# srogatch/ProbQA

Hardware: AMD Instinct MI355X
Metric: next_question_selections_per_sec (higher is better)
Workload: dtype f64; 1 GPU; 1000Qx5Ax1000T fp64 cube resident in HBM, single in-flight quiz; step = priority sweep + argmax + question id on host, synchronous call through the C ABI; questions_per_gpu=1000, parallelism=single GPU, eval_kernel=wg256_np2, selected_question=500

## Files before the change

probqa_amd/csrc/engine_options.h:

```cpp
#pragma once

#include <cstdint>
#include <cstdio>
#include <cstdlib>
#include <cstring>

#include "pqa_kernels.h"

namespace pqa {

struct EngineOptions {
  int64_t server = 0;
  int64_t serverIdleUs = 500;
  int64_t serverVramMailbox = 1;
  int64_t bugCompat = 1;
  int64_t speculate = 1;
  int64_t fuseUpdate = 1;
  int64_t combine = 1;
  int64_t combineSpin = 1;
  int64_t lingerUs = 20;
  int64_t postAlways = 0;
  int64_t poleFix = 1;
  int64_t poleGate = 1;
  int64_t poleLazy = 1;
  int64_t poleFollow = 1;
  int64_t lateEager = 3;
  int64_t select = 0;
  int64_t workers = 16;
  int64_t evalSubtasks = 0;
  int64_t evalVariant = 0;
  int64_t evalMaxGrid = 0;
  int64_t useGraph = 0;
  int64_t timeSweeps = 0;
  int64_t hostSampled = 1;
  int64_t fusedSampled = 0;
  int64_t sampledBatchHost = 0;
  int64_t batchMin = 0;
  int64_t batchForm = 0;
  int64_t batchQb = 0;
  int64_t batchTile = 0;
  int64_t batchGroups = 0;
  int64_t batchTail = 1;
  int64_t rerank = 1;
  int64_t clusterFrom = 10240;
  int64_t clusterForm = 0;
  int64_t clusterShape = 0;
  int64_t longRowForm = 1;
  int64_t topExact = 1;
  int64_t topCache = 10;
  int64_t rowsStage = 1;
  int64_t trainChunkSteps = int64_t(1) << 22;
};

enum : uint8_t {
// ... 106 lines not shown
```

probqa_amd/csrc/eval_kernels.hip:

```cpp
#include "pqa_device.h"
#include "eval_device.h"
#include "pqa_kernels.h"
#include "prior_device.h"
#include "pole_device.h"

namespace pqa {

static __device__ double gLog2Table[kLog2TableDoubles];
hipError_t UploadLog2Table(const double *hostTable) {
  return hipMemcpyToSymbol(HIP_SYMBOL(gLog2Table), hostTable, kLog2TableDoubles * sizeof(double));
}

struct EvalArgs {
  const double *cube;
  const double *prior;
  const uint32_t *tgap;
  const uint32_t *qgap;
  const uint32_t *asked;
  double *priority;
  double *poleScratch;
  PoleHeader *poleList;
  bool serverWatch;
  bool serverNoWatch;
  int64_t K, T, ldT, qFirst, qLimit;
  double vCompTail;
  FusedSelect fs;
  const QuizSlot *slots;
  int maxGrid;
  int poleNoFollow;
  int poleGate;
  const double *updRowA, *updRowD;
  int64_t updQuestion;
  int64_t updVects, updWorkers;
  int64_t updT;
  TopRequest updTop;
};

__device__ __forceinline__ void select_quiz(EvalArgs &a) {
  if (a.slots == nullptr) return;
  const QuizSlot s = a.slots[blockIdx.y];
  a.prior = s.prior;
  a.asked = s.asked;
  a.priority = s.priority;
  a.fs.out = s.out;
  a.fs.seq = s.seq;
  a.fs.hostPriority = s.hostPriority;
  a.fs.scratch += (size_t)blockIdx.y * (size_t)a.fs.scratchStride;
}

__device__ __forceinline__ void store_priority(double *p, double v) {
  __hip_atomic_store(p, v, __ATOMIC_RELAXED, __HIP_MEMORY_SCOPE_AGENT);
}

// ... 10 lines not shown
}
template <int CTRL>
__device__ __forceinline__ void best_step(Best &b) {
  const double op = mov_dpp<CTRL>(b.p);
  const int64_t oi = mov_dpp_i64<CTRL>(b.i);
  best_merge(b, op, oi);
}
__device__ __forceinline__ Best wave_best(Best b) {
  best_step<kDppXor1>(b);
  best_step<kDppXor2>(b);
  best_step<kDppHalfMirror>(b);
  best_step<kDppMirror>(b);
  Pair p = swap16(b.p);
  PairI64 i = swap16_i64(b.i);
  b = Best{p.a, i.a};
  best_merge(b, p.b, i.b);
  p = swap32(b.p);
  i = swap32_i64(b.i);
  b = Best{p.a, i.a};
  best_merge(b, p.b, i.b);
  return b;
}

template <bool UNI = false>
__device__ __forceinline__ void fused_select(const EvalArgs &a, Best mine, int lane, bool *allReported = nullptr, bool wgSuspect = false) {
  if (a.fs.scratch == nullptr) return;
  const bool sampled = a.fs.sampleSubtasks > 0;
  if (sampled && a.fs.hostPriority == nullptr) asm volatile("s_waitcnt vmcnt(0)" ::: "memory");
  const Best wg = wave_best(mine);
  uint64_t seqValue = a.fs.seqValue, flagValue = a.fs.flagValue;
  if (a.fs.tagCell != nullptr)
    seqValue = flagValue = __hip_atomic_load(a.fs.tagCell, __ATOMIC_RELAXED, __HIP_MEMORY_SCOPE_AGENT);
  const uint64_t tag = (uint64_t)(uint32_t)seqValue << 32;
  SelectResult *rec = a.fs.scratch;
  if (UNI || lane == 0) {
    typedef unsigned int u4 __attribute__((ext_vector_type(4)));
    const uint64_t w0 = d2u(wg.p), w1 = tag | (uint32_t)(wg.i < 0 ? 0x7FFFFFFFu : (uint32_t)wg.i) | (wgSuspect ? 0x80000000u : 0u);
    const u4 v = {(unsigned)w0, (unsigned)(w0 >> 32), (unsigned)w1, (unsigned)(w1 >> 32)};
    asm volatile("global_store_dwordx4 %0, %1, off sc1" ::"v"(rec + blockIdx.x), "v"(v) : "memory");
  }
  if (blockIdx.x != 0) return;
  const unsigned grid = gridDim.x;
  typedef unsigned int u4 __attribute__((ext_vector_type(4)));
  bool complete = true;
  uint32_t anySuspect = 0;
  Best b{0.0, -1};
  for (unsigned chunk = 0; chunk < grid && complete; chunk += 16 * kWave) {
// ... 13 lines not shown
          "s_waitcnt vmcnt(0)"
          : "=&v"(r[0]), "=&v"(r[1]), "=&v"(r[2]), "=&v"(r[3]), "=&v"(r[4]), "=&v"(r[5]), "=&v"(r[6]), "=&v"(r[7]),
            "=&v"(r[8]), "=&v"(r[9]), "=&v"(r[10]), "=&v"(r[11]), "=&v"(r[12]), "=&v"(r[13]), "=&v"(r[14]), "=&v"(r[15])
          : "v"(p0), "v"(p1), "v"(p2), "v"(p3)
          : "memory");
      bool mine = true;
#pragma unroll
      for (int u = 0; u < 16; u++)
        if (chunk + lane + u * kWave < grid) mine = mine && r[u][3] == (unsigned)(tag >> 32);
      all = __all(mine);
      if (!all) __builtin_amdgcn_s_sleep(2);
    }
    complete = all;
#pragma unroll
    for (int u = 0; u < 16; u++)
      if (chunk + lane + u * kWave < grid) {
        const uint64_t pw = (uint64_t)r[u][0] | ((uint64_t)r[u][1] << 32);
        anySuspect |= r[u][2] >> 31;
        best_merge(b, u2d(pw), (r[u][2] & 0x7FFFFFFFu) == 0x7FFFFFFFu ? -1 : (int64_t)(r[u][2] & 0x7FFFFFFFu));
      }
  }
  b = wave_best(b);
  const bool suspects = __any(anySuspect != 0);
  const bool listed = !UNI && suspects && complete && a.poleList != nullptr, lazy = a.fs.lazyFix != 0;
  const bool deferred = listed && !lazy, redo = (UNI && suspects && !a.serverNoWatch) || (listed && lazy);
  if (sampled) {
    if (allReported != nullptr && (UNI || lane == 0)) { allReported[0] = complete; allReported[1] = deferred; allReported[2] = redo; }
    return;
  }
  if (deferred) return;
  if (UNI || lane == 0) {
    if (a.fs.packed) host_publish_packed(a.fs.out, b.i < 0 ? 0.0 : b.p, flagValue, !complete ? -3 : redo ? -4 : b.i < 0 ? -1 : b.i);
    else host_publish(a.fs.out, b.i < 0 ? 0.0 : b.p, !complete ? -3 : redo ? -4 : b.i < 0 ? -1 : b.i + a.fs.outBase, a.fs.seq, flagValue);
    if (a.fs.tagCell != nullptr) {
      uint64_t next = seqValue + 1;
      if ((uint32_t)next == 0) next++;
      __hip_atomic_store(a.fs.tagCell, next, __ATOMIC_RELAXED, __HIP_MEMORY_SCOPE_AGENT);
    }
  }
}


constexpr int kSusDoubles = 4;

constexpr int kPend = 32;

__host__ __device__ constexpr size_t eval_lds_fixed_doubles(int wpq, int64_t K) {
  return kLog2TableDoubles + 2 * (size_t)wpq + 2 * (size_t)(K + 2) * wpq + (size_t)kPend * (2 * (size_t)K + 3) + 2 * kWave + kSusDoubles;
}
static_assert(kSusDoubles % 2 == 0 && kLog2TableDoubles % 2 == 0 && (kPend * 3) % 2 == 0,
              "the LDS priors behind the fixed part are read as 16-byte pairs: an odd count of doubles in front of them halves their rate (10000 x 5 x 10000: 906 -> 1250 us)");
__host__ __device__ constexpr size_t eval_md_row_offset_bytes(int wpq, int64_t K) {
  return (eval_lds_fixed_doubles(wpq, K) * sizeof(double) + 1023) / 1024 * 1024;
}
__host__ __device__ constexpr size_t eval_lds_doubles(int wpq, int64_t K, bool prLds, int64_t ldT) {
  return kLog2TableDoubles + 2 * (size_t)wpq + 2 * (size_t)(K + 2) * wpq + (size_t)kPend * (2 * (size_t)K + 3) + 2 * kWave + kSusDoubles +
         (prLds ? (size_t)ldT + 2 : 0);
}

__host__ __device__ constexpr bool eval_defers_sums(int wpq, int np, bool prLds) { return wpq <= 8 && !(wpq == 2 && np == 4); }
__host__ __device__ constexpr size_t eval_deferred_bytes(int wpq, int np, int64_t K, bool prLds) {
  return eval_defers_sums(wpq, np, prLds) ? (size_t)(K + 2) * wpq * kWave * sizeof(double) : 0;
}

__device__ __forceinline__ void flush_pending(const EvalArgs &a, const double *pend, int nPend, int lane, Best &best) {
  if (lane < nPend) {
    const int64_t K = a.K;
    const double *rec = pend + (size_t)lane * (2 * K + 3);
    const int64_t q = reinterpret_cast<const int64_t *>(rec)[2 * K + 2];
    const double pri = eval_epilogue(rec, -rec[2 * K], rec + K, K, rec[2 * K + 1], a.vCompTail);
    store_priority(a.priority + (q - a.qFirst), pri);
    if (a.fs.hostPriority != nullptr && a.fs.sampleSubtasks > 0) {
      typedef unsigned int u4 __attribute__((ext_vector_type(4)));
      const uint64_t w0 = d2u(pri), w1 = a.fs.seqValue;
      const u4 x = {(unsigned)w0, (unsigned)(w0 >> 32), (unsigned)w1, (unsigned)(w1 >> 32)};
      asm volatile("global_store_dwordx4 %0, %1, off sc0 sc1" ::"v"(a.fs.hostPriority + (q - a.qFirst)), "v"(x) : "memory");
    }
    best_offer(best, pri, q - a.qFirst);
  }
}

__device__ __forceinline__ double uniform_double(double x) {
  const uint64_t u = d2u(x);
  const uint32_t lo = __builtin_amdgcn_readfirstlane((uint32_t)u), hi = __builtin_amdgcn_readfirstlane((uint32_t)(u >> 32));
  return u2d(((uint64_t)hi << 32) | lo);
}
template <bool COH>
__device__ __forceinline__ uint32_t load_word(const uint32_t *p) {
  if constexpr (COH) return __hip_atomic_load(p, __ATOMIC_RELAXED, __HIP_MEMORY_SCOPE_AGENT);
  else return *p;
}
template <bool COH>
__device__ __forceinline__ double2 load_pair(const double2 *p) {
  if constexpr (COH) {
    const double *d = reinterpret_cast<const double *>(p);
    return make_double2(__hip_atomic_load(d, __ATOMIC_RELAXED, __HIP_MEMORY_SCOPE_AGENT),
                        __hip_atomic_load(d + 1, __ATOMIC_RELAXED, __HIP_MEMORY_SCOPE_AGENT));
  } else {
    return *p;
  }
}

template <int WPQ, int NP, bool PRLDS, bool SERVER, bool DEFER, bool FUSE = false, bool POLE = false, int KC = 0>
__device__ __forceinline__ void sweep_body(EvalArgs a, bool copyTable) {
  constexpr int kThreads = WPQ * kWave;
  constexpr int NPR = PRLDS ? 1 : NP;
  constexpr bool kStreamHint = !SERVER && WPQ >= 8;
  extern __shared__ double smem[];
  const int64_t ldT = a.ldT, K = KC > 0 ? KC : a.K;
  double *tbl = smem;
  if (!lds_table_at_zero(tbl)) __builtin_trap();
  double *redW = tbl + kLog2TableDoubles;
  double *partAll = redW + 2 * WPQ;
  double *pend = partAll + 2 * (K + 2) * WPQ;
  Best *bestLds = reinterpret_cast<Best *>(pend + kPend * (2 * K + 3));
  uint32_t *susWords = reinterpret_cast<uint32_t *>(bestLds + kWave);
  double2 *prLds = reinterpret_cast<double2 *>(reinterpret_cast<double *>(bestLds + kWave) + kSusDoubles);
  constexpr bool kMdLds = !PRLDS;
  double2 *mdRow = reinterpret_cast<double2 *>(reinterpret_cast<char *>(smem) + eval_md_row_offset_bytes(WPQ, K));
  const int nPart = (int)(K + 2);
  const int recLen = (int)(2 * K + 3);
  int tidRaw = threadIdx.x;
  if constexpr (SERVER) asm volatile("" : "+v"(tidRaw));
  const int tid = tidRaw, lane = tid % kWave;
  const int wave = SERVER ? (int)__builtin_amdgcn_readfirstlane(tid / kWave) : tid / kWave;
  const unsigned mdRowWaveAddr = (unsigned)(uintptr_t)mdRow + (unsigned)wave * 1024u;
  constexpr bool kDefer = DEFER;
  double *vdump = PRLDS ? reinterpret_cast<double *>(prLds) + ldT + 2
                        : reinterpret_cast<double *>(reinterpret_cast<char *>(mdRow) + (size_t)NP * kThreads * 16);
  const int nPairs = (int)(ldT >> 1);
  const int64_t qStride = (K + 1) * ldT, rowBytes = ldT * 8;
  uint32_t poff[NP];
  uint32_t gapWord[NP];
  double2 pr[NPR], prRaw[NP];
  double2 invD[NP], ring[NP];
  const int64_t q0 = a.qFirst + blockIdx.x;
  const bool haveQ0 = q0 < a.qLimit;
  const int64_t q0c = haveQ0 ? q0 : a.qLimit - 1;
  const uint32_t q0Gap = a.qgap[q0c >> 5], q0Asked = load_word<SERVER>(a.asked + (q0c >> 5));
#pragma unroll
  for (int j = 0; j < NP; j++) {
    const int p = tid + j * kThreads;
    const int pc = p < nPairs ? p : (nPairs - 1);
    poff[j] = (uint32_t)pc * 16u;
    gapWord[j] = a.tgap[pc >> 4];
    prRaw[j] = load_pair<SERVER>(reinterpret_cast<const double2 *>(a.prior) + pc);
  }
  auto head_of_stream = [&](int64_t qq) __attribute__((always_inline)) {
    if constexpr (kMdLds) {
      const RowRsrc rowA = row_rsrc(a.cube + qq * qStride, rowBytes);
      const dma_rsrc_t md = dma_rsrc<true>(a.cube + qq * qStride + K * ldT, rowBytes);
#pragma unroll
      for (int j = 0; j < NP; j++) {
        ring[j] = row_load<kStreamHint>(rowA, poff[j]);
        dma16(md, poff[j], mdRowWaveAddr + (unsigned)j * (kThreads * 16u));
      }
    } else {
      const RowRsrc rowD = row_rsrc(a.cube + qq * qStride + K * ldT, rowBytes);
#pragma unroll
      for (int j = 0; j < NP; j++) ring[j] = row_load<kStreamHint>(rowD, poff[j]);
    }
  };
// ... 36 lines not shown
#pragma unroll
    for (int j = 0; j < NP; j++) {
      const int p = tid + j * kThreads;
      if (p < nPairs) {
        double2 v = make_double2(stage[2 * p], stage[2 * p + 1]);
        if (2 * p < 4 * a.updVects) v.x = v.x / total;
        if (2 * p + 1 < 4 * a.updVects) v.y = v.y / total;
        prRaw[j] = v;
        if (blockIdx.x == gridDim.x - 1) { stage[2 * p] = v.x; stage[2 * p + 1] = v.y; }
      }
    }
    if (blockIdx.x == gridDim.x - 1) {
      if (tid == 0) const_cast<uint32_t *>(a.asked)[a.updQuestion >> 5] |= 1u << (a.updQuestion & 31);
      if (a.updTop.count > 0) {
        __syncthreads();
        top_targets_publish<true>(stage, a.tgap, a.updT, a.updTop.count, a.updTop.out, a.updTop.nOut, a.updTop.flag, a.updTop.flagValue, topScratch);
      }
    }
    __syncthreads();
    double2 *tblDst = reinterpret_cast<double2 *>(tbl);
    tblDst[tid] = tv0; tblDst[tid + kThreads] = tv1; tblDst[tid + 2 * kThreads] = tv2; tblDst[tid + 3 * kThreads] = tv3;
  }
  uint32_t gapBits = 0;
#pragma unroll
  for (int j = 0; j < NP; j++) {
    const int p = tid + j * kThreads;
    const bool inRow = p < nPairs;
    const int sh = (2 * (inRow ? p : nPairs - 1)) & 31;
    const bool g0 = !inRow || ((gapWord[j] >> sh) & 1u), g1 = !inRow || ((gapWord[j] >> (sh + 1)) & 1u);
    gapBits |= (g0 ? 1u : 0u) << (2 * j) | (g1 ? 1u : 0u) << (2 * j + 1);
    double2 pv = prRaw[j];
    pv.x = g0 ? 0.0 : pv.x;
    pv.y = g1 ? 0.0 : pv.y;
    if constexpr (PRLDS) { if (inRow) prLds[p] = pv; } else { pr[j] = pv; }
  }
  if constexpr (PRLDS) { if (tid == 0) prLds[nPairs] = make_double2(0.0, 0.0); }

  auto next_valid = [&](int64_t q) {
    while (q < a.qLimit && (bit_test(a.qgap, q) || ((load_word<SERVER>(a.asked + (q >> 5)) >> (q & 31)) & 1u) || (FUSE && q == a.updQuestion))) {
      if (tid == 0) store_priority(a.priority + (q - a.qFirst), 0.0);
      q += gridDim.x;
    }
    return q;
  };
  if (tid < 4) susWords[tid] = tid < 2 ? 0u : kGapNoneBits;
  int64_t q = q0;
  if (haveQ0 && ((((q0Gap | q0Asked) >> (q0 & 31)) & 1u) || (FUSE && q0 == a.updQuestion))) {
    q = next_valid(q0);
    if (q < a.qLimit) head_of_stream(q);
  }
  __syncthreads();

  int phase = 0, qpar = 0, nPend = 0;
  constexpr bool kWatch = POLE;
  constexpr bool kListWatch = kWatch && !SERVER;
  [[maybe_unused]] int32_t stepNear = INT32_MIN, stepSmall = INT32_MIN;
  const bool watchOn = SERVER ? a.serverWatch : a.poleList != nullptr;
  bool wgSuspect = false;
  if (wave == 0) bestLds[lane] = Best{0.0, -1};
  constexpr bool kHeadInTail = !kMdLds && KC > 0;
  [[maybe_unused]] bool firstOfStream = true;
  auto head_pair = [&](const RowRsrc &rowA, int j) __attribute__((always_inline)) {
    invD[j].x = ((gapBits >> (2 * j)) & 1) ? 0.0 : div_nr(1.0, ring[j].x);
    invD[j].y = ((gapBits >> (2 * j + 1)) & 1) ? 0.0 : div_nr(1.0, ring[j].y);
    ring[j] = row_load<kStreamHint>(rowA, poff[j]);
  };
  auto head_from_ring = [&](const double *qBase) __attribute__((always_inline)) {
    const RowRsrc rowA = row_rsrc(qBase, rowBytes);
#pragma unroll
    for (int j = 0; j < NP; j++) {
      head_pair(rowA, j);
      __builtin_amdgcn_sched_barrier(0);
    }
  };
  while (q < a.qLimit) {
    const int64_t qn = next_valid(q + gridDim.x);
    const double *qBase = a.cube + q * qStride;
    if constexpr (kMdLds) {
      asm volatile("s_waitcnt vmcnt(0)" ::: "memory");
#pragma unroll
      for (int j = 0; j < NP; j++) {
        const double2 dv = mdRow[j * kThreads + tid];
        invD[j].x = ((gapBits >> (2 * j)) & 1) ? 0.0 : div_nr(1.0, dv.x);
        invD[j].y = ((gapBits >> (2 * j + 1)) & 1) ? 0.0 : div_nr(1.0, dv.y);
        __builtin_amdgcn_sched_barrier(0);
      }
    } else if (!kHeadInTail || firstOfStream) {
      head_from_ring(qBase);
      firstOfStream = false;
    }
    double *part = partAll + qpar * (nPart * WPQ);
    double *rec = pend + nPend * recLen;
    double accL = 0, hW = 0;
    [[maybe_unused]] int32_t rowGap = INT32_MIN;
    [[maybe_unused]] uint32_t watchRows = 0;
#pragma unroll KC > 0 ? KC : 1
    for (int64_t k = 0; k < K; k++) {
      double2 lh[NP];
      double s0 = 0, s1 = 0;
      const bool lastRow = k + 1 == K;
      const bool moreQuestions = qn < a.qLimit;
      const double *rowNext = !lastRow ? qBase + (k + 1) * ldT
                              : !moreQuestions ? a.prior
                              : a.cube + qn * qStride + (kMdLds ? 0 : K * ldT);
      const RowRsrc rowN = row_rsrc(rowNext, rowBytes);
#pragma unroll
      for (int j = 0; j < NP; j++) {
// ... 85 lines not shown
        double acc = src[0];
#pragma unroll
        for (int i = 1; i < kGroups; i++) acc += src[32 * i];
        acc += mov_dpp<kDppXor1>(acc);
        acc += mov_dpp<kDppXor2>(acc);
        acc += mov_dpp<kDppHalfMirror>(acc);
        acc += mov_dpp<kDppMirror>(acc);
        const Pair p = swap16(acc);
        acc = p.a + p.b;
        if constexpr (kListWatch) {
          if (l32 == 0 && r < K && acc <= kSmallV && ((wideRows >> (r < 15 ? r : 15)) & 1u)) atomicOr(&susWords[qpar], 1u << (r < 15 ? r : 15));
        }
        if (r < K) acc = rec[r] * sqrt(acc);
        if (l32 == 0) rec[K + r] = acc;
      }
      if constexpr (kListWatch) {
        if (wideRows != 0) { __syncthreads(); suspect = (susWords[qpar] & 0xFFFFu) != 0; }
        if constexpr (!SERVER) { if (a.poleNoFollow) suspect = false; }
      }
      if (tid == 0) {
        reinterpret_cast<int64_t *>(rec)[2 * K + 2] = q;
        if constexpr (kListWatch) { susWords[qpar ^ 1] = 0; susWords[2 + (qpar ^ 1)] = kGapNoneBits; }
        if constexpr (!SERVER) {
          if (suspect) susWords[4] = pole_list_append(a.poleList, (uint32_t)(q - a.qFirst), K <= 15 ? susWords[qpar] & 0xFFFFu : 0u, a.slots != nullptr ? blockIdx.y : 0u,
                                                      a.poleGate ? susWords[2 + qpar] : 0u);
        }
      }
      wgSuspect = wgSuspect || suspect;
      if (!SERVER && suspect) {
        __syncthreads();
        const int64_t at = a.slots != nullptr ? (int64_t)susWords[4] : q - a.qFirst;
        for (int i = tid; i < 2 * (int)K + 2; i += kThreads) a.poleScratch[at * (2 * K + 2) + i] = rec[i];
      }
      if (nPend + 1 == kPend) {
        __syncthreads();
        if (wave == 0) flush_pending(a, pend, kPend, lane, bestLds[lane]);
      }
    } else {
      hW = wave_sum(hW);
      accL = wave_sum(accL);
      if (lane == 0) {
        part[K * WPQ + wave] = hW;
        part[(K + 1) * WPQ + wave] = accL;
      }
      if constexpr (kListWatch) {
        if (watchRows != 0) atomicOr(&susWords[qpar], watchRows);
      }
      if constexpr (WPQ > 1) __syncthreads();
      uint32_t wideRows = 0;
      if constexpr (kListWatch) {
        const uint32_t w = watchOn ? susWords[qpar] : 0u;
        suspect = (w & 0xFFFFu) != 0;
        wideRows = w >> 16;
      }
      if (wave == 0) {
        for (int r = lane; r < nPart; r += kWave) {
          double acc = part[r * WPQ];
          for (int w2 = 1; w2 < WPQ; w2++) acc += part[r * WPQ + w2];
          if constexpr (kListWatch) {
            if (r < K && acc <= kSmallV && ((wideRows >> (r < 15 ? r : 15)) & 1u)) atomicOr(&susWords[qpar], 1u << (r < 15 ? r : 15));
          }
          if (r < K) acc = rec[r] * sqrt(acc);
          rec[K + r] = acc;
        }
        if constexpr (kListWatch) { if (wideRows != 0) suspect = (susWords[qpar] & 0xFFFFu) != 0; }
        if constexpr (kListWatch && !SERVER) { if (a.poleNoFollow) suspect = false; }
        if (lane == 0) {
          reinterpret_cast<int64_t *>(rec)[2 * K + 2] = q;
          if constexpr (kListWatch) { susWords[qpar ^ 1] = 0; susWords[2 + (qpar ^ 1)] = kGapNoneBits; }
          if constexpr (!SERVER) {
            if (suspect) susWords[4] = pole_list_append(a.poleList, (uint32_t)(q - a.qFirst), K <= 15 ? susWords[qpar] & 0xFFFFu : 0u, a.slots != nullptr ? blockIdx.y : 0u,
                                                        a.poleGate ? susWords[2 + qpar] : 0u);
          }
        }
        wgSuspect = wgSuspect || suspect;
        if (!SERVER && suspect) {
          const int64_t at = a.slots != nullptr ? (int64_t)susWords[4] : q - a.qFirst;
          for (int i = lane; i < 2 * (int)K + 2; i += kWave) a.poleScratch[at * (2 * K + 2) + i] = rec[i];
        }
        if (nPend + 1 == kPend) flush_pending(a, pend, kPend, lane, bestLds[lane]);
      }
    }
    nPend = nPend + 1 == kPend ? 0 : nPend + 1;
    qpar ^= 1;
    q = qn;
  }
  if constexpr (kWatch && SERVER) { if (stepNear >= -0x00001000 || stepSmall >= -0x00201000) susWords[0] = 1u; }
  if constexpr (kDefer || (kWatch && SERVER)) __syncthreads();
  if constexpr (kWatch && SERVER) {
    if (wave == 0) { wgSuspect = watchOn && susWords[0] != 0u; if (lane == 0) susWords[0] = 0u; }
  }
  bool *allReported = reinterpret_cast<bool *>(redW);
  if (wave == 0) flush_pending(a, pend, nPend, lane, bestLds[lane]);
  if (wave == 0) fused_select<SERVER>(a, bestLds[lane], lane, allReported, wgSuspect);
  if constexpr (FUSE) {
    if (blockIdx.x == 0) {
      __syncthreads();
#pragma unroll
      for (int j = 0; j < NP; j++) {
        const int p = tid + j * kThreads;
        if (p < nPairs) reinterpret_cast<double2 *>(const_cast<double *>(a.prior))[p] = pr[j];
      }
    }
  }
  if (a.fs.scratch != nullptr && a.fs.sampleSubtasks > 0 && a.fs.hostPriority != nullptr) {
    if (blockIdx.x == 0) {
      __syncthreads();
      const bool complete = allReported[0], deferred = allReported[1], redo = allReported[2];
      if (!deferred && (SERVER ? wave == 0 : tid == 0)) {
        if (a.fs.packed) host_publish_packed(a.fs.out, 0.0, a.fs.flagValue, !complete ? -3 : redo ? -4 : 0);
        else host_publish(a.fs.out, 0.0, !complete ? -3 : redo ? -4 : 0, a.fs.seq, a.fs.flagValue);
      }
    }
    return;
  }
  if constexpr (!SERVER) {
    if (a.fs.scratch != nullptr && a.fs.sampleSubtasks > 0 && blockIdx.x == 0) {
      __syncthreads();
      const bool complete = allReported[0];
      if (allReported[1]) return;
      const SampledPick r = select_sampled_wg_lds<true>(a.priority, a.qgap, a.asked, a.qFirst, a.qLimit - a.qFirst,
                                                        a.fs.sampleSubtasks, a.fs.sampleRnd, tbl);
      if (tid == 0) {
        if (a.fs.packed) host_publish_packed(a.fs.out, r.priority, a.fs.flagValue, complete ? r.index : -3);
        else host_publish(a.fs.out, r.priority, complete ? r.index + a.fs.outBase : -3, a.fs.seq, a.fs.flagValue);
      }
    }
  }
}

template <int WPQ, int NP, bool PRLDS, bool DEFER, bool POLE = false, int KC = 0>
__global__ __launch_bounds__(WPQ * 64) void eval_questions_f64(EvalArgs a) {
  select_quiz(a);
  sweep_body<WPQ, NP, PRLDS, false, DEFER, false, POLE, KC>(a, true);
}
template <int WPQ, int NP, bool PRLDS, bool DEFER, bool POLE = false>
__global__ __launch_bounds__(WPQ * 64) __attribute__((amdgpu_waves_per_eu(3, 3))) void eval_questions_f64_occ3(EvalArgs a) {
  select_quiz(a);
  sweep_body<WPQ, NP, PRLDS, false, DEFER, false, POLE>(a, true);
}

template <int WPQ, int NP, bool DEFER, bool POLE = false, int KC = 0>
__global__ __launch_bounds__(WPQ * 64) void eval_questions_f64_upd(EvalArgs a) {
  sweep_body<WPQ, NP, false, false, DEFER, true, POLE, KC>(a, true);
}

__device__ __forceinline__ uint64_t uniform64(uint64_t x) {
  const uint32_t lo = __builtin_amdgcn_readfirstlane((uint32_t)x), hi = __builtin_amdgcn_readfirstlane((uint32_t)(x >> 32));
  return ((uint64_t)hi << 32) | lo;
}
static_assert(offsetof(ServerMailbox, stop) == 56 && offsetof(ServerMailbox, state) == 64 && sizeof(ServerCtl) == 64, "request line");
__device__ __forceinline__ uint64_t line_u64(uint32_t v, int i) {
  return (uint64_t)(uint32_t)__builtin_amdgcn_readlane((int)v, 2 * i) |
         ((uint64_t)(uint32_t)__builtin_amdgcn_readlane((int)v, 2 * i + 1) << 32);
}

template <int WPQ, int NP, bool DEFER, int KC>
__global__ __launch_bounds__(WPQ * 64) __attribute__((amdgpu_waves_per_eu(3, 3)))
void eval_server_f64(EvalArgs a, ServerMailbox *mb, uint32_t *requestLine, int everyonePolls, ServerCtl *ctl, uint64_t lastSeq,
                     uint64_t idleTicks, unsigned stepOffsetBytes) {
  extern __shared__ double smem[];
  uint32_t *step = reinterpret_cast<uint32_t *>(reinterpret_cast<char *>(smem) + stepOffsetBytes);
// ... 443 lines not shown
static bool eval_gates(const EvalArgs &args) {
  return args.poleGate && args.poleList != nullptr && args.slots == nullptr && args.fs.scratch != nullptr && args.fs.sampleSubtasks == 0 &&
         args.fs.hostPriority == nullptr && !args.poleNoFollow && args.ldT > 1024;
}
hipError_t launch_pole_fixup(const EvalArgs &args, hipStream_t stream, int nBatch = 1) {
  PoleFix f = PoleFixWV(args.cube, args.tgap, args.qgap, args.K, args.T, args.ldT);
  f.asked = args.asked; f.prior = args.prior;
  f.list = args.poleList; f.sums = args.poleScratch;
  f.priority = args.priority;
  f.qFirst = args.qFirst; f.nQ = args.qLimit - args.qFirst;
  f.capacity = f.nQ;
  f.vCompTail = args.vCompTail;
  f.fs = args.fs;
  if (args.fs.scratch != nullptr && args.fs.sampleSubtasks > 0 && args.fs.hostPriority != nullptr) { f.hostPriority = args.fs.hostPriority; f.hostTag = args.fs.seqValue; }
  f.gate = eval_gates(args) ? 1 : 0;
  if (args.slots != nullptr) {
    f.slots = args.slots; f.nSlots = nBatch; f.bySlot = 1; f.prior = nullptr; f.asked = nullptr; f.priority = nullptr;
    f.capacity = f.nQ * (int64_t)nBatch;
    f.hostTag = args.fs.seqValue;
  }
  return LaunchPoleFixup(f, stream);
}

template <int WPQ, int NP, bool PRLDS, bool DEFER, bool POLE = false, int KC = 0>
hipError_t launch_reg_form(const EvalArgs &args, int64_t nQ, int nBatch, hipStream_t stream) {
  if constexpr (!POLE) {
    if (args.poleList != nullptr) return launch_reg_form<WPQ, NP, PRLDS, DEFER, true, KC>(args, nQ, nBatch, stream);
  }
  if constexpr (KC == 0 && DEFER && NP != 4 && (!PRLDS || (WPQ == 8 && NP == 10))) {
    if (args.K == 5) return launch_reg_form<WPQ, NP, PRLDS, DEFER, POLE, 5>(args, nQ, nBatch, stream);
  }
  const size_t shmem = eval_base_lds_bytes<WPQ, NP, PRLDS>(args.K, args.ldT) + (DEFER ? eval_deferred_bytes(WPQ, NP, args.K, PRLDS) : 0);
  auto kern = [] {
    if constexpr (NP == 4 && WPQ == 4 && (DEFER || POLE)) return eval_questions_f64_occ3<WPQ, NP, PRLDS, DEFER, POLE>;
    else return eval_questions_f64<WPQ, NP, PRLDS, DEFER, POLE, KC>;
  }();
  static LaunchCache cache;
  const int dev = DeviceSlot();
  int perCU = 0;
  const hipError_t e = cache.Residency(dev, kern, WPQ * 64, shmem, &perCU);
  if (e != hipSuccess) return e;
  if (NP <= 2 && perCU > 3) perCU = 3;
  const int64_t resident = (int64_t)DeviceCUs(dev) * perCU;
  int64_t resGrid = nQ < resident ? nQ : resident;
  const int64_t maxRecords = args.slots != nullptr ? args.fs.scratchStride : kFusedMaxGrid;
  if (args.fs.scratch != nullptr && resGrid > maxRecords) resGrid = maxRecords;
  if (args.maxGrid > 0 && resGrid > args.maxGrid) resGrid = args.maxGrid;
  hipLaunchKernelGGL(kern, dim3((unsigned)resGrid, (unsigned)nBatch), dim3(WPQ * 64), shmem, stream, args);
  const hipError_t le = hipGetLastError();
  if constexpr (POLE) { if (le == hipSuccess && !args.poleNoFollow && !args.fs.lazyFix) return launch_pole_fixup(args, stream, nBatch); }
  return le;
}

template <int WPQ, int NP, bool PRLDS>
hipError_t launch_reg(const EvalArgs &args, int64_t nQ, int nBatch, hipStream_t stream) {
  if constexpr (eval_defers_sums(WPQ, NP, PRLDS)) {
    if (eval_base_lds_bytes<WPQ, NP, PRLDS>(args.K, args.ldT) + eval_deferred_bytes(WPQ, NP, args.K, PRLDS) <= kLdsPerCU)
      return launch_reg_form<WPQ, NP, PRLDS, true>(args, nQ, nBatch, stream);
  }
  return launch_reg_form<WPQ, NP, PRLDS, false>(args, nQ, nBatch, stream);
}

hipError_t launch_variant(const EvalArgs &args, int64_t ldT, int variant, int nBatch, hipStream_t stream) {
// ... 29 lines not shown
  const int v = pick_variant(kb.ldT, variant);
  for (const Variant &x : kVariants)
    if (x.id == v) return x.name;
  return "unknown";
}

static EvalArgs make_args(const KbView &kb, int64_t qFirst, int64_t qLimit) {
  EvalArgs args{};
  args.cube = static_cast<const double *>(kb.cube);
  args.tgap = kb.tgap;
  args.qgap = kb.qgap;
  args.K = kb.K;
  args.T = kb.T;
  args.ldT = kb.ldT;
  args.poleScratch = kb.poleScratch;
  args.poleList = kb.poleScratch != nullptr ? kb.poleList : nullptr;
  args.qFirst = qFirst;
  args.qLimit = qLimit;
  args.vCompTail = VCompTail(kb);
  args.fs = FusedSelect{};
  args.slots = nullptr;
  args.maxGrid = kb.maxGrid;
  args.poleNoFollow = kb.poleNoFollow;
  args.poleGate = kb.poleGate;
  return args;
}
static void finish_args(EvalArgs &args) { args.poleGate = eval_gates(args) ? 1 : 0; }

hipError_t LaunchEvalQuestions(const KbView &kb, const double *prior, const uint32_t *asked, int64_t qFirst,
                               int64_t qLimit, double *priority, int variant, const FusedSelect *fused,
                               hipStream_t stream) {
  if (qLimit <= qFirst) return hipSuccess;
  EvalArgs args = make_args(kb, qFirst, qLimit);
  args.prior = prior;
  args.asked = asked;
  args.priority = priority;
  if (fused) args.fs = *fused;
  finish_args(args);
  return launch_variant(args, kb.ldT, variant, 1, stream);
}

hipError_t LaunchEvalPoleFixup(const KbView &kb, const double *prior, const uint32_t *asked, double *priority, const FusedSelect &fused,
                               hipStream_t stream) {
  EvalArgs args = make_args(kb, 0, kb.Q);
  if (args.poleList == nullptr) return hipErrorInvalidValue;
  args.prior = prior;
// ... 138 lines not shown
```

probqa_amd/csrc/hip_engine.cpp:

```cpp
#include "hip_engine_internal.h"

namespace pqa {

const char *ErrCodeName(ErrCode c) {
  switch (c) {
    case ErrCode::None: return "Success";
    case ErrCode::NotImplemented: return "Not implemented";
    case ErrCode::SRException: return "SRException";
    case ErrCode::StdException: return "std::exception";
    case ErrCode::InsufficientEngineDimensions: return "Insufficient engine dimensions";
    case ErrCode::MaintenanceModeChangeInProgress: return "Maintenance mode change is in progress";
    case ErrCode::MaintenanceModeAlreadyThis: return "Maintenance mode is already this";
    case ErrCode::ObjectShutDown: return "Object is shut(ting) down";
    case ErrCode::IndexOutOfRange: return "Index is out of range";
    case ErrCode::Aggregate: return "Aggregate error";
    case ErrCode::NegativeCount: return "The count is negative";
    case ErrCode::NonPositiveAmount: return "The amount is not positive";
    case ErrCode::AbsentId: return "The ID is absent from KB";
    case ErrCode::WrongMode: return "An attempt to execute an operation in a wrong mode";
    case ErrCode::UnhandledCase: return "Unhandled case";
    case ErrCode::I64Underflow: return "Underflow of a 64-bit integer";
    case ErrCode::QuestionsExhausted: return "Engine has run out of questions";
    case ErrCode::NoQuizActiveQuestion: return "No active question in the quiz";
    case ErrCode::CantOpenFile: return "Cannot open file";
// ... 282 lines not shown
  StopServer();
  _kbVersion++;
  for (Quiz *q : _quizzes) if (q) q->topOp = 0;
  HIP_TRY(hipMemcpyAsync(_dTGap, _hTGap.data(), _hTGap.size() * sizeof(uint32_t), hipMemcpyHostToDevice, _stream));
  HIP_TRY(hipMemcpyAsync(_dQGap, _hQGap.data(), _hQGap.size() * sizeof(uint32_t), hipMemcpyHostToDevice, _stream));
  HIP_TRY(hipStreamSynchronize(_stream));
  return Error();
}

KbView HipEngine::View() const {
  KbView v;
  v.cube = _dCube; v.elem = _elem; v.vB = _dVB; v.tgap = _dTGap; v.qgap = _dQGap;
  v.K = _K; v.Q = _Q; v.T = _T; v.ldT = _ldT;
  v.nValidTargets = _T - _nTargetGaps;
  v.smallLaunches = _opt.server ? 1 : 0;
  v.priorScratch = _opt.longRowForm ? _dPriorScratch : nullptr;
  v.maxGrid = (int)_opt.evalMaxGrid;
  v.clusterForm = (int)_opt.clusterForm;
  v.clusterShape = (int)_opt.clusterShape;
  v.clusterFrom = ClusterFrom();
  v.poleScratch = _opt.poleFix ? _dPoleScratch : nullptr;
  v.poleNoFollow = _opt.poleFollow ? 0 : 1;
  v.poleGate = _opt.poleFix && _opt.poleGate ? 1 : 0;
  v.poleList = _opt.poleFix ? reinterpret_cast<PoleHeader *>(_dPoleScratch + (size_t)_capQ * (size_t)(2 * _K + 2)) : nullptr;
  return v;
}

Error HipEngine::SetOption(const char *name, int64_t value) {
  std::lock_guard<EngineMutex> lk(_mu);
  const std::string n(name ? name : "");
  (void)FlushUpdates();
  if (n == "seed") { _rng.Seed((uint64_t)value); return Error(); }
  const OptionSpec *o = FindOption(n.c_str());
  const auto is = [o](int64_t EngineOptions::*field) { return o->field == field; };
  if (!o || !AcceptOption(*o, value) || (is(&EngineOptions::serverVramMailbox) && _serverStream))
    return Error::Make(ErrCode::UnhandledCase, "Unknown option or value out of range: " + n);
  if (is(&EngineOptions::speculate)) DropSpeculation();
  if (o->effects & kOptStopServer) StopServer();
  if (o->effects & kOptSettlePoleList) (void)SettlePoleList();
  _opt.*o->field = value;
  if (o->effects & kOptBumpKbVersion) _kbVersion++;
  if (is(&EngineOptions::speculate)) _specScore = 0;
  if (is(&EngineOptions::topCache)) _topWantRecent = value;
  return Error();
}

int64_t HipEngine::GetOption(const char *name) const {
  const std::string n(name ? name : "");
  if (const OptionSpec *o = FindOption(n.c_str())) {
    const auto is = [o](int64_t EngineOptions::*field) { return o->field == field; };
    if (is(&EngineOptions::evalSubtasks)) return _opt.evalSubtasks ? _opt.evalSubtasks : 8 * _opt.workers;
    if (is(&EngineOptions::serverVramMailbox) && _serverStream) return _serverRequestInVram ? 1 : 0;
    if (is(&EngineOptions::evalMaxGrid)) return -1;
    return _opt.*o->field;
  }
  static constexpr struct { const char *name; uint64_t HipEngine::*counter; } kCounters[] = {
      {"sampled_batches", &HipEngine::_sampledBatches},
      {"sampled_batch_device_ns", &HipEngine::_sampledBatchDeviceNs},
      {"priority_host_bytes", &HipEngine::_priorityHostBytes},
      {"among_calls", &HipEngine::_amongCalls},
      {"among_pairs", &HipEngine::_amongPairs},
      {"preview_calls", &HipEngine::_previewCalls},
      {"preview_pairs", &HipEngine::_previewPairs},
      {"preview_device_ns", &HipEngine::_previewDeviceNs},
      {"review_calls", &HipEngine::_reviewCalls},
      {"review_rows", &HipEngine::_reviewRows},
      {"review_device_ns", &HipEngine::_reviewDeviceNs},
      {"status_calls", &HipEngine::_statusCalls},
      {"status_quizzes", &HipEngine::_statusQuizzes},
      {"rank_calls", &HipEngine::_rankCalls},
      {"rank_pairs", &HipEngine::_rankPairs},
      {"status_device_ns", &HipEngine::_statusDeviceNs},
      {"gain_calls", &HipEngine::_gainCalls},
      {"gain_quizzes", &HipEngine::_gainQuizzes},
      {"gain_device_ns", &HipEngine::_gainDeviceNs},
      {"page_calls", &HipEngine::_pageCalls},
      {"page_quizzes", &HipEngine::_pageQuizzes},
      {"page_device_ns", &HipEngine::_pageDeviceNs},
// ... 509 lines not shown
```

probqa_amd/csrc/pqa_kernels.h:

```cpp
#pragma once

#include <hip/hip_runtime.h>
#include <stdint.h>

#include <atomic>

#include "select_record.h"

namespace pqa {

constexpr size_t kLdsPerCU = 160 * 1024;
constexpr size_t kLdsNoOptIn = 64 * 1024;
constexpr double kLnSqrt2 = 0.34657359027997265470861606072909;

constexpr int kMaxDevices = 64;
inline int DeviceSlot() { int d = 0; return hipGetDevice(&d) == hipSuccess ? (d & (kMaxDevices - 1)) : 0; }
inline int DeviceCUs(int dev) {
  static std::atomic<int> numCUs[kMaxDevices];
  int n = numCUs[dev].load(std::memory_order_relaxed);
  if (n == 0) {
    int d = 0;
    n = (hipGetDevice(&d) == hipSuccess && hipDeviceGetAttribute(&n, hipDeviceAttributeMultiprocessorCount, d) == hipSuccess && n > 0) ? n : 256;
    numCUs[dev].store(n, std::memory_order_relaxed);
  }
// ... 38 lines not shown
    if (e == hipSuccess) Put(dev, key, 1);
    return e;
  }
};

struct KbView {
  const void *cube;
  int elem;
  const double *vB;
  const uint32_t *tgap;
  const uint32_t *qgap;
  int64_t K, Q, T, ldT;
  int64_t nValidTargets;
  int smallLaunches;
  double *priorScratch;
  int maxGrid;
  int clusterForm;
  int clusterShape;
  int64_t clusterFrom;
  double *poleScratch;
  struct PoleHeader *poleList;
  int poleNoFollow;
  int poleGate;
};

inline double VCompTail(const KbView &kb) {
  const double nT = (double)(kb.nValidTargets + 1);
  return kLnSqrt2 / (nT * nT);
}

struct PoleHeader { uint32_t count, arrived; unsigned long long floorBits; };
struct PoleEntry {
  uint32_t q;
  uint32_t rowMask;
  uint32_t b;
  uint32_t gap;
};
static_assert(sizeof(PoleHeader) == 16, "header and entries are 16 bytes each");
size_t PoleListBytes(int64_t capacity);
hipError_t UploadLog2TablePole(const double *hostTable);

struct SelectResult {
  double priority;
  int64_t index;
};

// ... 456 lines not shown
```

probqa_amd/csrc/sharded_engine.cpp:

```cpp
#include "hip_engine_internal.h"

#include <unordered_set>

namespace pqa {

namespace {

Error NotSharded(const char *what) {
  return Error::MakeP(ErrCode::NotImplemented, std::string("Feature=") + what + " on a sharded engine",
                      std::string(what) + " is not available when the question axis is split over several devices (PQA_DEVICES).");
}

struct alignas(64) Slot {
  double priority;
  int64_t index;
  uint64_t flag;
};

}

class ShardedEngine final : public IEngine {
 public:
  static ShardedEngine *Create(Error &err, const CiEngineDefinition &def, const std::vector<int> &devices);
  ~ShardedEngine() override;
// ... 1419 lines not shown
    for (int64_t q = 0; q < nLocal; q++) {
      const int64_t old = srcQ[(size_t)(first + q)];
      if (old < 0) continue;
      const int owner = OwnerOf(old);
      blocks[(size_t)q] = _sh[(size_t)owner]->QuestionBlock(old - _sh[(size_t)owner]->FirstQuestion());
    }
    err = e->AdoptRows(blocks, s0.RowLength(), srcT, _sh[(size_t)s]->VBDevicePtr());
    if (!err.ok()) return err;
    std::vector<int64_t> localQ;
    std::vector<double> localInit;
    for (size_t i = 0; i < fillQ.size(); i++)
      if (fillQ[i] >= first && fillQ[i] < first + nLocal) { localQ.push_back(fillQ[i] - first); localInit.push_back(fillQInit[i]); }
    err = e->ApplyFills(fillT, fillTInit, localQ, localInit);
    if (!err.ok()) return err;
    err = e->SetQuestionGaps((int64_t)qGaps.size(), qGaps.data());
    if (err.ok()) err = e->SetTargetGaps((int64_t)tGaps.size(), tGaps.data());
    if (!err.ok()) return err;
    e->SetTargetIds(targetIds);
    e->SetQuizIds(_sh[(size_t)s]->QuizIds());
    Error ae;
    e->SetQuestionsAsked(s == 0 ? s0.GetTotalQuestionsAsked(ae) : 0);
    for (const char *opt : {"select", "workers", "eval_subtasks", "eval_variant", "bug_compat", "top_cache", "speculate", "host_sampled",
                            "fused_sampled", "batch_min", "batch_qb", "batch_tile", "batch_groups", "batch_tail", "batch_form", "cluster_form", "cluster_shape", "rerank", "combine", "server", "use_graph",
                            "pole_fix", "pole_lazy", "late_eager", "long_row_form", "fuse_update", "combine_spin", "combine_linger_us", "post_always", "server_idle_us"}) {
      const int64_t v = _sh[(size_t)s]->GetOption(opt);
      if (v >= 0) (void)e->SetOption(opt, std::string(opt) == "eval_subtasks" && v == 8 * _sh[(size_t)s]->GetOption("workers") ? 0 : v);
    }
    err = e->StartMaintenance(false);
    if (!err.ok()) return err;
  }
  _sh.swap(fresh);
  _Q = newQ;
  _T = newT;
  _qGapList = qGaps;
  _hostPriority.assign((size_t)newQ, 0.0);
  ForgetQuizzes();
  RefreshGapBits();
  AdoptShards();
  std::fill(_remoteReads.begin(), _remoteReads.end(), 0);
  std::fill(_trainEpoch.begin(), _trainEpoch.end(), 0);
  std::fill(_seenTrain.begin(), _seenTrain.end(), 0);
  return Error();
}

Error ShardedEngine::AddQsTs(int64_t nQuestions, CiAddQorTParam *pAqps, int64_t nTargets, CiAddQorTParam *pAtps) {
  std::lock_guard<OpLock> lk(_opMu);
  Error e = _sh[0]->IsMaintenanceMode() ? Error() : WrongModeErr("add questions/targets");
// ... 122 lines not shown
```

Before: 43920 selections/s.

## Add specialized lone-sweep kernel variant for single-quiz K=5 register-prior sweeps

Adds a dedicated eval kernel instantiation for the common case: no quiz slots, no sampling, pole list on, K=5, WPQ=4, NP=2. It constant-folds the unused paths and reloads rarely used pointers from the kernarg segment instead of holding them in registers. It also masks the inverse denominators with precomputed bitmasks instead of selects, and skips next_valid for the first step using a prefetched gap/asked word. The goal is lower register pressure and less scalar and branch work per sweep, at the cost of more code paths and a separate residency cache. The new path is enabled by default through a new lone_sweep option.

```diff
diff --git a/probqa_amd/csrc/engine_options.h b/probqa_amd/csrc/engine_options.h
--- a/probqa_amd/csrc/engine_options.h
+++ b/probqa_amd/csrc/engine_options.h
@@ -30,6 +30,7 @@
   int64_t evalSubtasks = 0;
   int64_t evalVariant = 0;
   int64_t evalMaxGrid = 0;
+  int64_t loneSweep = 1;
   int64_t useGraph = 0;
   int64_t timeSweeps = 0;
   int64_t hostSampled = 1;
diff --git a/probqa_amd/csrc/eval_kernels.hip b/probqa_amd/csrc/eval_kernels.hip
--- a/probqa_amd/csrc/eval_kernels.hip
+++ b/probqa_amd/csrc/eval_kernels.hip
@@ -29,6 +29,7 @@
   int maxGrid;
   int poleNoFollow;
   int poleGate;
+  int lone;
   const double *updRowA, *updRowD;
   int64_t updQuestion;
   int64_t updVects, updWorkers;
@@ -85,7 +86,7 @@
   return b;
 }
 
-template <bool UNI = false>
+template <bool UNI = false, bool LISTS = false>
 __device__ __forceinline__ void fused_select(const EvalArgs &a, Best mine, int lane, bool *allReported = nullptr, bool wgSuspect = false) {
   if (a.fs.scratch == nullptr) return;
   const bool sampled = a.fs.sampleSubtasks > 0;
@@ -145,7 +146,7 @@
   }
   b = wave_best(b);
   const bool suspects = __any(anySuspect != 0);
-  const bool listed = !UNI && suspects && complete && a.poleList != nullptr, lazy = a.fs.lazyFix != 0;
+  const bool listed = !UNI && suspects && complete && (LISTS || a.poleList != nullptr), lazy = a.fs.lazyFix != 0;
   const bool deferred = listed && !lazy, redo = (UNI && suspects && !a.serverNoWatch) || (listed && lazy);
   if (sampled) {
     if (allReported != nullptr && (UNI || lane == 0)) { allReported[0] = complete; allReported[1] = deferred; allReported[2] = redo; }
@@ -186,12 +187,24 @@
   return eval_defers_sums(wpq, np, prLds) ? (size_t)(K + 2) * wpq * kWave * sizeof(double) : 0;
 }
 
+__device__ __forceinline__ double and_words(double x, uint32_t m) {
+  const uint64_t u = d2u(x);
+  return u2d((uint64_t)((uint32_t)(u >> 32) & m) << 32 | (uint64_t)((uint32_t)u & m));
+}
+template <typename T>
+__device__ __forceinline__ T kernarg_member(size_t offset) {
+  const char __attribute__((address_space(4))) *p = (const char __attribute__((address_space(4))) *)__builtin_amdgcn_kernarg_segment_ptr();
+  asm volatile("" : "+s"(p));
+  return *reinterpret_cast<const T __attribute__((address_space(4))) *>(p + offset);
+}
+
+template <bool LONE = false>
 __device__ __forceinline__ void flush_pending(const EvalArgs &a, const double *pend, int nPend, int lane, Best &best) {
   if (lane < nPend) {
     const int64_t K = a.K;
     const double *rec = pend + (size_t)lane * (2 * K + 3);
     const int64_t q = reinterpret_cast<const int64_t *>(rec)[2 * K + 2];
-    const double pri = eval_epilogue(rec, -rec[2 * K], rec + K, K, rec[2 * K + 1], a.vCompTail);
+    const double pri = eval_epilogue(rec, -rec[2 * K], rec + K, K, rec[2 * K + 1], LONE ? kernarg_member<double>(offsetof(EvalArgs, vCompTail)) : a.vCompTail);
     store_priority(a.priority + (q - a.qFirst), pri);
     if (a.fs.hostPriority != nullptr && a.fs.sampleSubtasks > 0) {
       typedef unsigned int u4 __attribute__((ext_vector_type(4)));
@@ -224,8 +237,15 @@
   }
 }
 
-template <int WPQ, int NP, bool PRLDS, bool SERVER, bool DEFER, bool FUSE = false, bool POLE = false, int KC = 0>
+template <int WPQ, int NP, bool PRLDS, bool SERVER, bool DEFER, bool FUSE = false, bool POLE = false, int KC = 0, bool LONE = false>
 __device__ __forceinline__ void sweep_body(EvalArgs a, bool copyTable) {
+  static_assert(!LONE || (!SERVER && !FUSE && !PRLDS && DEFER && POLE), "the lone form: a launched, watching, deferred-sums sweep of a register-prior shape");
+  if constexpr (LONE) {
+    a.slots = nullptr;
+    a.fs.sampleSubtasks = 0; a.fs.hostPriority = nullptr; a.fs.tagCell = nullptr; a.fs.packed = 1; a.fs.outBase = 0;
+    a.poleGate = 0; a.poleNoFollow = 0;
+    if constexpr (KC > 0) a.K = KC;
+  }
   constexpr int kThreads = WPQ * kWave;
   constexpr int NPR = PRLDS ? 1 : NP;
   constexpr bool kStreamHint = !SERVER && WPQ >= 8;
@@ -261,6 +281,11 @@
   const bool haveQ0 = q0 < a.qLimit;
   const int64_t q0c = haveQ0 ? q0 : a.qLimit - 1;
   const uint32_t q0Gap = a.qgap[q0c >> 5], q0Asked = load_word<SERVER>(a.asked + (q0c >> 5));
+  [[maybe_unused]] uint32_t q1Words = 0;
+  if constexpr (LONE) {
+    const int64_t q1 = q0 + gridDim.x, q1c = q1 < a.qLimit ? q1 : a.qLimit - 1;
+    q1Words = a.qgap[q1c >> 5] | a.asked[q1c >> 5];
+  }
 #pragma unroll
   for (int j = 0; j < NP; j++) {
     const int p = tid + j * kThreads;
@@ -343,6 +368,7 @@
     tblDst[tid] = tv0; tblDst[tid + kThreads] = tv1; tblDst[tid + 2 * kThreads] = tv2; tblDst[tid + 3 * kThreads] = tv3;
   }
   uint32_t gapBits = 0;
+  [[maybe_unused]] uint32_t keep[2 * NP];
 #pragma unroll
   for (int j = 0; j < NP; j++) {
     const int p = tid + j * kThreads;
@@ -354,7 +380,9 @@
     pv.x = g0 ? 0.0 : pv.x;
     pv.y = g1 ? 0.0 : pv.y;
     if constexpr (PRLDS) { if (inRow) prLds[p] = pv; } else { pr[j] = pv; }
-  }
+    if constexpr (LONE) { keep[2 * j] = g0 ? 0u : ~0u; keep[2 * j + 1] = g1 ? 0u : ~0u; }
+  }
+  if constexpr (LONE) { for (int i = 0; i < 2 * NP; i++) asm volatile("" : "+v"(keep[i])); }
   if constexpr (PRLDS) { if (tid == 0) prLds[nPairs] = make_double2(0.0, 0.0); }
 
   auto next_valid = [&](int64_t q) {
@@ -376,7 +404,7 @@
   constexpr bool kWatch = POLE;
   constexpr bool kListWatch = kWatch && !SERVER;
   [[maybe_unused]] int32_t stepNear = INT32_MIN, stepSmall = INT32_MIN;
-  const bool watchOn = SERVER ? a.serverWatch : a.poleList != nullptr;
+  const bool watchOn = LONE ? true : SERVER ? a.serverWatch : a.poleList != nullptr;
   bool wgSuspect = false;
   if (wave == 0) bestLds[lane] = Best{0.0, -1};
   constexpr bool kHeadInTail = !kMdLds && KC > 0;
@@ -394,16 +422,27 @@
       __builtin_amdgcn_sched_barrier(0);
     }
   };
+  if constexpr (LONE) asm volatile("" : "+v"(q1Words));
   while (q < a.qLimit) {
-    const int64_t qn = next_valid(q + gridDim.x);
+    int64_t qn = q + gridDim.x;
+    if (LONE && q == a.qFirst + blockIdx.x) {
+      if (qn < a.qLimit && ((__builtin_amdgcn_readfirstlane(q1Words) >> (qn & 31)) & 1u)) qn = next_valid(qn);
+    } else {
+      qn = next_valid(qn);
+    }
     const double *qBase = a.cube + q * qStride;
     if constexpr (kMdLds) {
       asm volatile("s_waitcnt vmcnt(0)" ::: "memory");
 #pragma unroll
       for (int j = 0; j < NP; j++) {
         const double2 dv = mdRow[j * kThreads + tid];
-        invD[j].x = ((gapBits >> (2 * j)) & 1) ? 0.0 : div_nr(1.0, dv.x);
-        invD[j].y = ((gapBits >> (2 * j + 1)) & 1) ? 0.0 : div_nr(1.0, dv.y);
+        if constexpr (LONE) {
+          invD[j].x = and_words(div_nr(1.0, dv.x), keep[2 * j]);
+          invD[j].y = and_words(div_nr(1.0, dv.y), keep[2 * j + 1]);
+        } else {
+          invD[j].x = ((gapBits >> (2 * j)) & 1) ? 0.0 : div_nr(1.0, dv.x);
+          invD[j].y = ((gapBits >> (2 * j + 1)) & 1) ? 0.0 : div_nr(1.0, dv.y);
+        }
         __builtin_amdgcn_sched_barrier(0);
       }
     } else if (!kHeadInTail || firstOfStream) {
@@ -535,19 +574,20 @@
         reinterpret_cast<int64_t *>(rec)[2 * K + 2] = q;
         if constexpr (kListWatch) { susWords[qpar ^ 1] = 0; susWords[2 + (qpar ^ 1)] = kGapNoneBits; }
         if constexpr (!SERVER) {
-          if (suspect) susWords[4] = pole_list_append(a.poleList, (uint32_t)(q - a.qFirst), K <= 15 ? susWords[qpar] & 0xFFFFu : 0u, a.slots != nullptr ? blockIdx.y : 0u,
-                                                      a.poleGate ? susWords[2 + qpar] : 0u);
+          if (suspect) susWords[4] = pole_list_append(LONE ? kernarg_member<PoleHeader *>(offsetof(EvalArgs, poleList)) : a.poleList, (uint32_t)(q - a.qFirst),
+                                                      K <= 15 ? susWords[qpar] & 0xFFFFu : 0u, a.slots != nullptr ? blockIdx.y : 0u, a.poleGate ? susWords[2 + qpar] : 0u);
         }
       }
       wgSuspect = wgSuspect || suspect;
       if (!SERVER && suspect) {
         __syncthreads();
         const int64_t at = a.slots != nullptr ? (int64_t)susWords[4] : q - a.qFirst;
-        for (int i = tid; i < 2 * (int)K + 2; i += kThreads) a.poleScratch[at * (2 * K + 2) + i] = rec[i];
+        double *sums = LONE ? kernarg_member<double *>(offsetof(EvalArgs, poleScratch)) : a.poleScratch;
+        for (int i = tid; i < 2 * (int)K + 2; i += kThreads) sums[at * (2 * K + 2) + i] = rec[i];
       }
       if (nPend + 1 == kPend) {
         __syncthreads();
-        if (wave == 0) flush_pending(a, pend, kPend, lane, bestLds[lane]);
+        if (wave == 0) flush_pending<LONE>(a, pend, kPend, lane, bestLds[lane]);
       }
     } else {
       hW = wave_sum(hW);
@@ -591,7 +631,7 @@
           const int64_t at = a.slots != nullptr ? (int64_t)susWords[4] : q - a.qFirst;
           for (int i = lane; i < 2 * (int)K + 2; i += kWave) a.poleScratch[at * (2 * K + 2) + i] = rec[i];
         }
-        if (nPend + 1 == kPend) flush_pending(a, pend, kPend, lane, bestLds[lane]);
+        if (nPend + 1 == kPend) flush_pending<LONE>(a, pend, kPend, lane, bestLds[lane]);
       }
     }
     nPend = nPend + 1 == kPend ? 0 : nPend + 1;
@@ -604,8 +644,11 @@
     if (wave == 0) { wgSuspect = watchOn && susWords[0] != 0u; if (lane == 0) susWords[0] = 0u; }
   }
   bool *allReported = reinterpret_cast<bool *>(redW);
-  if (wave == 0) flush_pending(a, pend, nPend, lane, bestLds[lane]);
-  if (wave == 0) fused_select<SERVER>(a, bestLds[lane], lane, allReported, wgSuspect);
+  int tidEnd = threadIdx.x;
+  if constexpr (LONE) asm volatile("" : "+v"(tidEnd));
+  const bool epilogueWave = LONE ? tidEnd / kWave == 0 : wave == 0;
+  if (epilogueWave) flush_pending<LONE>(a, pend, nPend, lane, bestLds[lane]);
+  if (epilogueWave) fused_select<SERVER, LONE>(a, bestLds[lane], lane, allReported, wgSuspect);
   if constexpr (FUSE) {
     if (blockIdx.x == 0) {
       __syncthreads();
@@ -651,6 +694,11 @@
 __global__ __launch_bounds__(WPQ * 64) __attribute__((amdgpu_waves_per_eu(3, 3))) void eval_questions_f64_occ3(EvalArgs a) {
   select_quiz(a);
   sweep_body<WPQ, NP, PRLDS, false, DEFER, false, POLE>(a, true);
+}
+
+template <int WPQ, int NP, int KC>
+__global__ __launch_bounds__(WPQ * 64) void eval_questions_f64_lone(EvalArgs a) {
+  sweep_body<WPQ, NP, false, false, true, false, true, KC, true>(a, true);
 }
 
 template <int WPQ, int NP, bool DEFER, bool POLE = false, int KC = 0>
@@ -1140,6 +1188,11 @@
   return LaunchPoleFixup(f, stream);
 }
 
+static bool eval_is_lone(const EvalArgs &args) {
+  return args.lone && args.slots == nullptr && (args.fs.scratch == nullptr || args.fs.packed) && args.fs.sampleSubtasks == 0 &&
+         args.fs.hostPriority == nullptr && args.fs.tagCell == nullptr && !args.poleGate && !args.poleNoFollow && args.poleList != nullptr;
+}
+
 template <int WPQ, int NP, bool PRLDS, bool DEFER, bool POLE = false, int KC = 0>
 hipError_t launch_reg_form(const EvalArgs &args, int64_t nQ, int nBatch, hipStream_t stream) {
   if constexpr (!POLE) {
@@ -1156,7 +1209,15 @@
   static LaunchCache cache;
   const int dev = DeviceSlot();
   int perCU = 0;
-  const hipError_t e = cache.Residency(dev, kern, WPQ * 64, shmem, &perCU);
+  if constexpr (WPQ == 4 && NP == 2 && !PRLDS && DEFER && POLE && KC == 5) {
+    if (eval_is_lone(args)) {
+      kern = eval_questions_f64_lone<WPQ, NP, KC>;
+      static LaunchCache loneCache;
+      const hipError_t e = loneCache.Residency(dev, kern, WPQ * 64, shmem, &perCU);
+      if (e != hipSuccess) return e;
+    }
+  }
+  const hipError_t e = perCU > 0 ? hipSuccess : cache.Residency(dev, kern, WPQ * 64, shmem, &perCU);
   if (e != hipSuccess) return e;
   if (NP <= 2 && perCU > 3) perCU = 3;
   const int64_t resident = (int64_t)DeviceCUs(dev) * perCU;
@@ -1232,6 +1293,7 @@
   args.slots = nullptr;
   args.maxGrid = kb.maxGrid;
   args.poleNoFollow = kb.poleNoFollow;
+  args.lone = kb.loneSweep;
   args.poleGate = kb.poleGate;
   return args;
 }
diff --git a/probqa_amd/csrc/hip_engine.cpp b/probqa_amd/csrc/hip_engine.cpp
--- a/probqa_amd/csrc/hip_engine.cpp
+++ b/probqa_amd/csrc/hip_engine.cpp
@@ -328,6 +328,7 @@
   v.poleScratch = _opt.poleFix ? _dPoleScratch : nullptr;
   v.poleNoFollow = _opt.poleFollow ? 0 : 1;
   v.poleGate = _opt.poleFix && _opt.poleGate ? 1 : 0;
+  v.loneSweep = _opt.loneSweep ? 1 : 0;
   v.poleList = _opt.poleFix ? reinterpret_cast<PoleHeader *>(_dPoleScratch + (size_t)_capQ * (size_t)(2 * _K + 2)) : nullptr;
   return v;
 }
@@ -337,6 +338,7 @@
   const std::string n(name ? name : "");
   (void)FlushUpdates();
   if (n == "seed") { _rng.Seed((uint64_t)value); return Error(); }
+  if (n == "lone_sweep") { StopServer(); _opt.loneSweep = value ? 1 : 0; return Error(); }
   const OptionSpec *o = FindOption(n.c_str());
   const auto is = [o](int64_t EngineOptions::*field) { return o->field == field; };
   if (!o || !AcceptOption(*o, value) || (is(&EngineOptions::serverVramMailbox) && _serverStream))
@@ -360,6 +362,7 @@
     if (is(&EngineOptions::evalMaxGrid)) return -1;
     return _opt.*o->field;
   }
+  if (n == "lone_sweep") return _opt.loneSweep;
   static constexpr struct { const char *name; uint64_t HipEngine::*counter; } kCounters[] = {
       {"sampled_batches", &HipEngine::_sampledBatches},
       {"sampled_batch_device_ns", &HipEngine::_sampledBatchDeviceNs},
diff --git a/probqa_amd/csrc/pqa_kernels.h b/probqa_amd/csrc/pqa_kernels.h
--- a/probqa_amd/csrc/pqa_kernels.h
+++ b/probqa_amd/csrc/pqa_kernels.h
@@ -84,6 +84,7 @@
   struct PoleHeader *poleList;
   int poleNoFollow;
   int poleGate;
+  int loneSweep;
 };
 
 inline double VCompTail(const KbView &kb) {
diff --git a/probqa_amd/csrc/sharded_engine.cpp b/probqa_amd/csrc/sharded_engine.cpp
--- a/probqa_amd/csrc/sharded_engine.cpp
+++ b/probqa_amd/csrc/sharded_engine.cpp
@@ -1465,7 +1465,7 @@
     e->SetQuestionsAsked(s == 0 ? s0.GetTotalQuestionsAsked(ae) : 0);
     for (const char *opt : {"select", "workers", "eval_subtasks", "eval_variant", "bug_compat", "top_cache", "speculate", "host_sampled",
                             "fused_sampled", "batch_min", "batch_qb", "batch_tile", "batch_groups", "batch_tail", "batch_form", "cluster_form", "cluster_shape", "rerank", "combine", "server", "use_graph",
-                            "pole_fix", "pole_lazy", "late_eager", "long_row_form", "fuse_update", "combine_spin", "combine_linger_us", "post_always", "server_idle_us"}) {
+                            "pole_fix", "pole_lazy", "lone_sweep", "late_eager", "long_row_form", "fuse_update", "combine_spin", "combine_linger_us", "post_always", "server_idle_us"}) {
       const int64_t v = _sh[(size_t)s]->GetOption(opt);
       if (v >= 0) (void)e->SetOption(opt, std::string(opt) == "eval_subtasks" && v == 8 * _sh[(size_t)s]->GetOption("workers") ? 0 : v);
     }
```

Result: no change. 43900 selections/s (median of 3 runs) (-0.1%).
